# revdotcom/reverb

Measured on AMD Instinct MI355X. Metric: RTFx (audio-sec/wall-sec) Reverb-ASR attention_rescoring, higher is better.
Workload: dtype bf16

## Files before the change

### reverb_amd/_lib.py

```python
from __future__ import annotations

import ctypes as C
import os

_HERE = os.path.dirname(os.path.abspath(__file__))
LIB_PATH = os.path.join(_HERE, "librvb.so")

RVB_F32, RVB_BF16, RVB_FP8 = 0, 1, 2
ACT_NONE, ACT_SILU, ACT_RELU = 0, 1, 2
NORM_LN, NORM_AFFINE = 0, 1


class RvbError(RuntimeError):
    pass


class AudioInfo(C.Structure):
    _fields_ = [("container", C.c_int32), ("sample_format", C.c_int32), ("channels", C.c_int32), ("sample_rate", C.c_int32),
                ("bits_per_sample", C.c_int32), ("md5_checked", C.c_int32), ("frames", C.c_int64), ("decode_threads", C.c_int32),
                ("reserved", C.c_int32)]


class _SizedCfg(C.Structure):

# ... 115 lines not shown
                [("p", _f32p), ("p_rows", C.c_int32), ("p_stride", C.c_int32), ("p_col", C.c_int32), ("p_off", C.c_int32),
                 ("bias_u", _f32p), ("bias_v", _f32p)] +
                [(n, _i32p) for n in ("q_start", "q_len", "kv_start", "kv_len", "q_pos0", "kv_index", "work")] +
                [(n, C.c_int32) for n in ("n_index", "n_work", "max_q", "q_block", "causal", "chunk", "left", "plain_order", "fold",
                                          "k_prefolded", "fold_kv_cap", "lab")] +
                [("ran", C.c_int32 * 8)])


class NormTestArgs(C.Structure):
    _fields_ = ([(n, C.c_int32) for n in ("dtype", "x_bf16", "mode", "silu", "out_f32", "out_fp8", "out2_fp8", "M", "d", "pad0")] +
                [(n, C.c_float) for n in ("eps", "eps2", "out_scale", "out2_scale")] +
                [(n, _f32p) for n in ("x", "gamma", "beta", "add", "gamma2", "beta2", "out", "out2")] +
                [("sat", C.c_uint32), ("sat2", C.c_uint32)])


class GemmTestArgs(C.Structure):
    _fields_ = ([(n, C.c_int32) for n in ("dtype", "M", "N", "K", "lda", "ldw", "ldc", "ldres", "act", "out_f32", "out_fp8", "in_fp8",
                                          "inplace", "a_row0", "c_rows", "conv", "cT1", "cF1", "cC", "cB")] +
                [(n, C.c_float) for n in ("alpha", "a_scale", "out_scale")] +
                [("path", C.c_int32), ("a_elems", C.c_int64)] +
                [(n, _f32p) for n in ("A", "W", "bias", "res", "C", "a_deq", "w_deq")])


_u32p = C.POINTER(C.c_uint32)

TEST_SIGNATURES = {
    "rvb_test_gemm_ex": (C.c_int, [C.POINTER(GemmTestArgs)]),
    "rvb_test_rownorm_ex": (C.c_int, [C.POINTER(NormTestArgs)]),
    "rvb_test_conv1_ex": (C.c_int, [C.c_int, _f32p, _f32p, _f32p, _f32p, _f32p, _f32p, C.c_int, C.c_int, C.c_int, C.c_int, C.c_float,
                                    _f32p, _u32p]),
    "rvb_test_embed": (C.c_int, [_f32p, C.c_int, _f32p, C.c_int, _i32p, _i32p, _f32p, C.c_int, C.c_int, C.c_float]),
    "rvb_test_amax_abs": (C.c_int, [C.c_int, _f32p, C.c_int64, _f32p]),
    "rvb_test_convert_f32": (C.c_int, [C.c_int, _f32p, _f32p, C.c_int64]),
    "rvb_test_gather_cache": (C.c_int, [C.c_void_p, C.c_void_p, _i32p, C.c_int, C.c_int, C.c_int, C.c_int]),
    "rvb_test_gather_pairs": (C.c_int, [_f32p, C.c_int, C.c_int64, _i32p, _i32p, C.c_int, _f32p]),
    "rvb_test_gemm": (C.c_int, [C.c_int, _f32p, _f32p, _f32p, _f32p, _f32p, C.c_int, C.c_int, C.c_int, C.c_float,
                                C.c_int, C.c_int, C.c_int, C.c_int, C.c_int, C.c_int, C.c_int]),
    "rvb_test_rownorm": (C.c_int, [C.c_int, _f32p, _f32p, _f32p, C.c_float, C.c_int, C.c_int, _f32p, _f32p, C.c_int,
                                   C.c_int, C.c_int]),
    "rvb_test_conv_block32": (C.c_int, [_f32p, _f32p, _f32p, _f32p, _f32p, _f32p, C.c_int, C.c_int, C.c_int]),
    "rvb_test_conv_s2sc": (C.c_int, [_f32p, _f32p, _f32p, _f32p, _f32p, _f32p, _f32p, C.c_int, C.c_int, C.c_int]),
    "rvb_test_conv1": (C.c_int, [C.c_int, _f32p, _f32p, _f32p, _f32p, _f32p, _f32p, C.c_int, C.c_int, C.c_int, C.c_int]),
    "rvb_test_conv_igemm_fp8": (C.c_int, [_f32p, _f32p, _f32p, _f32p, _f32p, _f32p, C.c_int, C.c_int, C.c_int, C.c_int, C.c_int, C.c_int, C.c_int,
                                           C.c_float, C.c_float, _f32p, _f32p, _f32p]),
    "rvb_test_joint_new": (C.c_void_p, [C.c_int, C.c_int, C.c_int, C.c_int, C.c_double, C.c_double, C.c_double]),
    "rvb_test_joint_free": (None, [C.c_void_p]),
    "rvb_test_joint_begin": (C.c_int, [C.c_void_p, C.c_int, _f32p, _i32p, C.c_int, C.c_float, C.c_float, _i32p, _i32p, _i32p, _i32p, _i32p,
                                       C.c_int]),
    "rvb_test_joint_finish": (C.c_int, [C.c_void_p, _f32p]),
    "rvb_test_joint_prefix": (C.c_int, [C.c_void_p, C.c_int, _i32p, _i32p]),
    "rvb_test_joint_result": (C.c_int, [C.c_void_p, _i32p, _i32p, _i32p, _f64p, _i32p, _f64p]),
    "rvb_test_glu_dwconv": (C.c_int, [C.c_int, _f32p, _f32p, _f32p, _f32p, _i32p, _f32p, C.c_int, C.c_int, C.c_int,
                                      C.c_int, C.c_int, _f32p, C.c_int]),
    "rvb_test_attention": (C.c_int, [C.c_int, _f32p, _f32p, _f32p, _f32p, _f32p, _f32p, _f32p, C.c_int, C.c_int,
                                     C.c_int, C.c_int, C.c_int, _i32p, _i32p, _i32p, _i32p, C.c_int, C.c_int]),
    "rvb_test_attention_trie": (C.c_int, [C.c_int, _f32p, _f32p, _f32p, _f32p, C.c_int, C.c_int, C.c_int, _i32p, _i32p, _i32p,
                                          _i32p, _i32p, _i32p, C.c_int, C.c_int, C.c_int]),
    "rvb_test_attention_ex": (C.c_int, [C.POINTER(AttnTestArgs)]),
    "rvb_test_attention_pos_bias": (C.c_int, [_f32p, C.c_int, C.c_int, C.c_int, C.c_int, _f32p, _f32p, C.c_int, C.c_int, C.c_float, _f32p]),
    "rvb_test_logsoftmax_topk": (C.c_int, [_f32p, C.c_int, C.c_int, C.c_int, C.c_float, C.c_int, _f32p, _i32p, _f32p]),
    "rvb_test_lse_gather": (C.c_int, [_f32p, C.c_int, C.c_int, _i32p, _f32p]),
    "rvb_test_logsoftmax_topk_ex": (C.c_int, [_f32p, C.c_int, C.c_int, C.c_int, C.c_int, C.c_float, C.c_int, _f32p, _i32p, _f32p]),
    "rvb_test_lse_gather_ex": (C.c_int, [_f32p, C.c_int, C.c_int, C.c_int, _i32p, C.c_float, C.c_int, _f32p]),
    "rvb_test_lse_gather_multi_ex": (C.c_int, [_f32p, C.c_int, C.c_int, C.c_int, _i32p, _i32p, _f32p]),
    "rvb_test_ctc_viterbi": (C.c_int, [_f32p, C.c_int, C.c_int, _i32p, C.c_int, C.c_int, C.c_int, _i32p, _f32p]),
    "rvb_test_ctc_viterbi_wild": (C.c_int, [_f32p, C.c_int, C.c_int, _f32p, C.c_float, _i32p, C.c_int, C.c_int, C.c_int, _i32p, _f32p]),
    "rvb_test_ctc_viterbi_graph": (C.c_int, [_f32p, _i32p, C.c_int, C.c_int, _f32p, C.c_float, _i32p, _i32p, _i32p, _i32p, _u8p, C.c_int,
                                             C.c_int, _i32p, _i32p, _f32p]),
    "rvb_test_ctc_score": (C.c_int, [_f32p, C.c_int, C.c_int, _i32p, C.c_int, C.c_int, C.c_int, _f64p, _f32p, _f32p, _f32p, _i32p]),
    "rvb_test_ctc_score_graph": (C.c_int, [_f32p, _i32p, C.c_int, C.c_int, _i32p, _i32p, _i32p, _i32p, _u8p, C.c_int, C.c_int, _f64p, _f32p,
                                           _f32p, _f32p, _f32p, _i32p]),
    "rvb_test_ctc_score_batch": (C.c_int, [_f32p, _i32p, C.c_int, _i32p, _i32p, C.c_int, C.c_int, C.c_int, _f64p, _f32p, _f32p, _f32p,
                                           _i32p]),
    "rvb_test_ctc_find": (C.c_int, [_f32p, _i32p, C.c_int, C.c_int, _f32p, _i32p, _i32p, C.c_int, _f32p, C.c_int, C.c_int, C.c_int, C.c_int,
                                    _i64p, _i32p, _i32p, _f32p, _i32p, _i32p, _i32p, _f32p]),
    "rvb_test_slab_windows": (C.c_int, [C.c_char_p, _i32p, _i32p, C.c_int, _i32p, C.c_int, C.c_int, _i32p, _i32p, _i32p, _i32p, _i32p]),
    "rvb_test_gemm_glu": (C.c_int, [_f32p, _f32p, _f32p, _f32p, C.c_int, C.c_int, C.c_int]),
    "rvb_test_gemm_rowadd": (C.c_int, [_f32p, _f32p, _f32p, _f32p, _f32p, C.c_int, C.c_int, C.c_int, C.c_int, C.c_int, C.c_int]),
    "rvb_test_mp3_decode": (C.c_int64, [C.c_char_p, C.c_int64, C.c_int, _f32p, C.c_int64, _i64p, _i64p, C.c_int]),
    "rvb_test_mp3_hybrid": (C.c_int, [_f32p, _f32p, C.c_int, C.c_int, _f32p]),
    "rvb_test_mp3_polyphase": (C.c_int, [_f32p, _f32p, _i32p, _f32p]),
    "rvb_test_mp3_window": (C.c_int, [_f32p]),
    "rvb_test_mp3_huffman": (C.c_int, [C.c_int, C.POINTER(C.c_uint16), C.POINTER(C.c_uint8), _i32p]),
    "rvb_test_gemm_fp8": (C.c_int, [_f32p, _f32p, _f32p, _f32p, _f32p, C.c_int, C.c_int, C.c_int, C.c_float, C.c_float, C.c_int, C.c_int,
                                    C.c_float, _f32p, _f32p]),
    "rvb_test_rownorm_fp8": (C.c_int, [_f32p, _f32p, _f32p, C.c_float, C.c_int, C.c_int, C.c_int, C.c_float, _f32p, _f32p, _f32p,
                                       C.c_float, C.c_float, _f32p, _f32p]),
    "rvb_test_lse_gather_multi": (C.c_int, [_f32p, C.c_int, C.c_int, _i32p, _i32p, C.c_int, _f32p]),
    "rvb_test_row_xent": (C.c_int, [_f32p, C.c_int, C.c_int, C.c_int, _i32p, _i32p, _f32p, _f32p, _f64p, _i32p]),
    "rvb_test_host_pool": (C.c_int, [C.c_int, C.c_int, C.c_int]),
    "rvb_test_build_trie": (C.c_int, [_i32p, _i32p, _i32p, C.c_int, C.c_int, C.c_int, C.c_int, C.c_int, _i32p, _i32p, _i32p, _i32p, _i32p, _i32p,
                                      _i32p, _i32p, _i32p, _i32p, _i32p]),
    "rvb_test_fbank": (C.c_int, [_i16p, C.c_int64, _f32p]),
    "rvb_test_fbank_ex": (C.c_int, [_i16p, _f32p, C.c_int64, _f32p]),
    "rvb_test_fbank_batch": (C.c_int, [C.POINTER(C.c_void_p), _i32p, _i64p, _i64p, C.c_int, C.c_int, _f32p]),
    "rvb_test_set_gemm_variant": (C.c_int, [C.c_int]),
    "rvb_test_set_gemm2_opts": (C.c_int, [C.c_int, C.c_int]),
    "rvb_test_gemm_timeline": (C.c_int, [C.c_int] * 6 + [C.POINTER(C.c_longlong), C.c_int, _i32p]),
    "rvb_test_gemm_bench": (C.c_int, [C.c_int, C.c_int, C.c_int, C.c_int, C.c_int, C.c_int, C.c_int, C.c_int, C.c_int,
                                      _f64p, _f64p]),
    "rvb_test_prefix_beam": (C.c_int, [_f32p, _i32p, C.c_int, C.c_int, C.c_int, _i32p, _i32p, _i32p, _i32p, _i32p,
                                       _f64p]),
    "rvb_test_prefix_beam_context": (C.c_int, [_f32p, _i32p, C.c_int, C.c_int, C.c_int, C.c_int, _i32p, _i32p, C.c_int, C.c_double,
                                               _i32p, _i32p, _i32p, _i32p, _i32p, _f64p, _f64p]),
    "rvb_test_context_walk": (C.c_int, [_i32p, _i32p, C.c_int, C.c_double, C.c_int, C.c_int, _i32p, C.c_int, _i32p, _f64p, _i32p,
                                        _f64p]),
# ... 127 lines not shown
```

### reverb_amd/csrc/elementwise.hip

```cpp
#include <algorithm>

#include "common.h"
#include "kernels.h"

namespace rvb {

static constexpr int CONV1_ROWS = 4;

template <typename T>
__global__ __launch_bounds__(256) void conv1_kernel(const float* __restrict__ feats, const float* __restrict__ mean,
                                                    const float* __restrict__ istd, const float* __restrict__ w,
                                                    const float* __restrict__ bias, T* __restrict__ out, int T0,
                                                    int F0, int T1, int F1, int d, float inv_scale, unsigned* __restrict__ amax,
                                                    unsigned* __restrict__ sat) {
  extern __shared__ float s_in[];
  const int t1_0 = blockIdx.x * CONV1_ROWS, b = blockIdx.y;
  const int nrow = min(CONV1_ROWS, T1 - t1_0);
  for (int i = threadIdx.x; i < (2 * nrow + 1) * F0; i += 256) {
    const int kh = i / F0, f = i - kh * F0;
    s_in[i] = (feats[((size_t)b * T0 + 2 * t1_0 + kh) * F0 + f] - mean[f]) * istd[f];
  }
  __syncthreads();
  const int ncg = d >> 3;
  const int per = ncg < 256 ? ncg : 256;
  const int nslots = 256 / per;
  const int cgl = threadIdx.x % per, fslot = threadIdx.x / per;
  if (fslot >= nslots) return;
  float vmax = 0.f;
  unsigned nclip = 0;
  for (int cg = cgl; cg < ncg; cg += per) {
    float wr[8][9], br[8];
#pragma unroll
    for (int k = 0; k < 9; ++k) {
      const float4 lo = *(const float4*)(w + (size_t)k * d + cg * 8), hi = *(const float4*)(w + (size_t)k * d + cg * 8 + 4);
      wr[0][k] = lo.x; wr[1][k] = lo.y; wr[2][k] = lo.z; wr[3][k] = lo.w;
      wr[4][k] = hi.x; wr[5][k] = hi.y; wr[6][k] = hi.z; wr[7][k] = hi.w;
    }
#pragma unroll
    for (int c = 0; c < 8; ++c) br[c] = bias[cg * 8 + c];
    for (int row = 0; row < nrow; ++row) {
      T* orow = out + ((size_t)b * T1 + t1_0 + row) * F1 * d;
      const float* in = s_in + 2 * row * F0;
      for (int f1 = fslot; f1 < F1; f1 += nslots) {
        float xin[9];
#pragma unroll
        for (int kh = 0; kh < 3; ++kh)
#pragma unroll
          for (int kw = 0; kw < 3; ++kw) xin[kh * 3 + kw] = in[kh * F0 + 2 * f1 + kw];
        float o[8];
        if constexpr (sizeof(T) == 4) {
#pragma unroll
          for (int c = 0; c < 8; ++c) {
            float acc = br[c];
// ... 416 lines not shown
    for (int e = 0; e < VE; ++e) sv[e] = Gate<T>::put(g[e]);
    uint4* dst = (uint4*)&s_g[r][grp * VE];
#pragma unroll
    for (int q = 0; q < (int)(VE * sizeof(S)) / 16; ++q) dst[q] = ((const uint4*)sv)[q];
  }
  }
  __syncthreads();
  if (!cok) return;
  constexpr int OPT = DW_TT / (DW_THREADS / 64);
  f32x2_t acc[OPT];
  const f32x2_t bv = {a.dw_b[ch], a.dw_b[ch + 1]};
#pragma unroll
  for (int i = 0; i < OPT; ++i) acc[i] = bv;
  const int rbase = slot * OPT;
#pragma unroll
  for (int r = 0; r < OPT + DW_KMAX - 1; ++r) {
    float gx, gy;
    Gate<T>::get(*(const typename Gate<T>::pair_t*)&s_g[rbase + r][2 * c], gx, gy);
    const f32x2_t g = {gx, gy};
#pragma unroll
    for (int i = 0; i < OPT; ++i) {
      const int k = r - i;
      if (k >= 0 && k < DW_KMAX) acc[i] = __builtin_elementwise_fma(wk[k], g, acc[i]);
    }
  }
#pragma unroll
  for (int i = 0; i < OPT; ++i) {
    const int t = t0 + rbase + i;
    if (t < a.T) {
      if (a.out_bf16) *(uint32_t*)((bf16_t*)a.out + ((size_t)b * a.T + t) * a.d + ch) = pack2_bf16(acc[i].x, acc[i].y);
      else *(float2*)(a.out + ((size_t)b * a.T + t) * a.d + ch) = make_float2(acc[i].x, acc[i].y);
    }
  }
}

int glu_dwconv(hipStream_t s, int dtype, const GluDwArgs& a) {
  if (a.B <= 0 || a.T <= 0) return OK;
  if (a.K > DW_KMAX || a.K < 1 || (!a.causal && (a.K % 2) == 0) || (a.d % 2)) {
    set_error("glu_dwconv: kernel must be <= 31 (and odd unless causal), d even"); return E_ARG;
  }
  if (a.gated && (a.hist_rows > 0 || (a.d % (dtype == DT_BF16 ? 8 : 4)) != 0)) {
    set_error("glu_dwconv: a gated input comes in whole 16-byte vectors and without a streaming history"); return E_ARG;
  }
  if (a.hist_rows > 0 && (!a.causal || a.B != 1 || a.hist_rows > a.K - 1 || !a.hist)) {
    set_error("glu_dwconv: a left-context history belongs to one causal stream"); return E_ARG;
  }
  dim3 grid(cdiv(a.T, DW_TT), cdiv(a.d, DW_CT), a.B);
  if (dtype == DT_BF16) hipLaunchKernelGGL(glu_dw_kernel<bf16_t>, grid, dim3(DW_THREADS), 0, s, a);
  else hipLaunchKernelGGL(glu_dw_kernel<float>, grid, dim3(DW_THREADS), 0, s, a);
  RVB_HIP_CHECK(hipGetLastError());
  return OK;
}

__global__ __launch_bounds__(256) void embed_kernel(const float* __restrict__ E, const float* __restrict__ pe,
                                                    const int* __restrict__ tok, const int* __restrict__ pos,
                                                    float* __restrict__ out, int rows, int d, float scale) {
  const int row = blockIdx.x;
  const float* e = E + (size_t)tok[row] * d;
  const float* p = pe + (size_t)pos[row] * d;
  for (int c = threadIdx.x; c < d; c += 256) out[(size_t)row * d + c] = e[c] * scale + p[c];
}

int embed_tokens(hipStream_t s, const float* E, const float* pe, const int* tok, const int* pos, float* out,
                 int rows, int d, float scale) {
  if (rows <= 0) return OK;
  hipLaunchKernelGGL(embed_kernel, dim3(rows), dim3(256), 0, s, E, pe, tok, pos, out, rows, d, scale);
  RVB_HIP_CHECK(hipGetLastError());
  return OK;
}

template <typename T>
__global__ __launch_bounds__(256) void amax_kernel(const T* __restrict__ x, size_t n, float* __restrict__ slot) {
  float m = 0.f;
  for (size_t i = (size_t)blockIdx.x * 256 + threadIdx.x; i < n; i += (size_t)gridDim.x * 256) m = fmaxf(m, fabsf(Cvt<T>::to_f32(x[i])));
  m = wave_max(m);
  if ((threadIdx.x & 63) == 0 && m > 0.f) atomicMax((unsigned int*)slot, __float_as_uint(m));
}
int amax_abs(hipStream_t s, int dtype, const void* x, size_t n, float* slot) {
  if (n == 0) return OK;
  const int blocks = (int)std::min<size_t>((n + 255) / 256, 2048);
  if (dtype == DT_BF16) hipLaunchKernelGGL(amax_kernel<bf16_t>, dim3(blocks), dim3(256), 0, s, (const bf16_t*)x, n, slot);
  else hipLaunchKernelGGL(amax_kernel<float>, dim3(blocks), dim3(256), 0, s, (const float*)x, n, slot);
  RVB_HIP_CHECK(hipGetLastError());
  return OK;
}

template <typename T>
__global__ __launch_bounds__(256) void convert_kernel(const float* __restrict__ src, T* __restrict__ dst, size_t n) {
  for (size_t i = (size_t)blockIdx.x * 256 + threadIdx.x; i < n; i += (size_t)gridDim.x * 256)
    dst[i] = Cvt<T>::from_f32(src[i]);
}

int convert_f32(hipStream_t s, int dtype, const float* src, void* dst, size_t n) {
  if (n == 0) return OK;
  const int blocks = (int)((n + 255) / 256 < 4096 ? (n + 255) / 256 : 4096);
  if (dtype == DT_BF16) hipLaunchKernelGGL(convert_kernel<bf16_t>, dim3(blocks), dim3(256), 0, s, src, (bf16_t*)dst, n);
  else hipLaunchKernelGGL(convert_kernel<float>, dim3(blocks), dim3(256), 0, s, src, (float*)dst, n);
  RVB_HIP_CHECK(hipGetLastError());
  return OK;
}

__global__ __launch_bounds__(256) void gather_cache_kernel(const char* __restrict__ src, char* __restrict__ dst,
                                                           const int* __restrict__ parent, int L, int rows, int row_bytes) {
  const int r = blockIdx.y;
  const size_t so = (size_t)parent[r] * L * row_bytes, dof = (size_t)r * L * row_bytes;
  const int nvec = rows * (row_bytes / 16);
// ... 15 lines not shown
```

### reverb_amd/csrc/engine_encode.hip

```cpp
#include "engine_impl.h"

#include <algorithm>
#include <cmath>
#include <cstdlib>
#include <cstring>

namespace rvb {

static constexpr int GLU_FUSE_DEFAULT = 1;

static int encoder_layer(rvb_engine* e, EncLayer& L, int lidx, int M, int B, int T, const LNorm& next, void* next_out,
                         float next8 = 0.f, int li = -1) {
  const int d = e->cfg.d_model, ff = e->cfg.ffn_dim, heads = e->cfg.heads, dk = d / heads;
  float* x = e->x.as<float>();
  const bool f8 = e->fp8 && e->f8_state == 2 && li < 0;
  const bool cal = e->fp8 && e->f8_state == 1 && li < 0;
  const unsigned grp = f8 ? e->f8_groups[lidx] : 0u;
  const bool f8_ffm = grp & 1u, f8_qkv = grp & 2u, f8_pw1 = grp & 4u, f8_pw2 = grp & 8u, f8_ff = (grp & 16u) && !L.is_lsl;
  const F8Scales sc8 = f8 ? e->f8[lidx] : F8Scales();
  const char* prefold_env = lab_env("RVB_ATTN_PREFOLD");
  const int prefold_on = prefold_env ? atoi(prefold_env) : 1;
  const bool prefold = prefold_on && e->dtype == DT_BF16 && li < 0 && !f8_qkv && L.pos_bias.p != nullptr && dk > 32 && dk <= 64 &&
                       T <= e->pe_rows && T <= 16384 && (d % 8) == 0;
  auto note = [&](int slot, const void* t, size_t n) -> int {
// ... 37 lines not shown
      static const int fold = lab_env("RVB_ATTN_FOLD") ? atoi(lab_env("RVB_ATTN_FOLD")) : 0;
      const int cap = (T + 63) / 64 * 64;
      if (fold && li < 0 && L.pos_bias.p && cap <= 16384) { a.pos_bias = L.pos_bias.as<float>(); a.pos_bias_stride = e->pe_rows; a.fold_kv_cap = cap; }
      if (prefold && cap <= 16384) { a.pos_bias = L.pos_bias.as<float>(); a.pos_bias_stride = e->pe_rows; a.k_prefolded = 1; a.fold_kv_cap = cap; }
    }
    a.q_stride = a.k_stride = a.v_stride = 3 * d; a.p_stride = d; a.o_stride = d;
    a.bias_u = L.bias_u.as<float>(); a.bias_v = L.bias_v.as<float>();
    a.out = e->ao.p;
    a.q_start = e->d_seq_start.as<int>(); a.q_len = e->d_seq_len.as<int>();
    a.kv_start = e->d_seq_start.as<int>(); a.kv_len = e->cur_lens;
    a.nseq = B; a.heads = heads; a.dk = dk; a.max_q = T; a.causal = 0; a.sqrt_dk = std::sqrt((float)dk);
    a.chunk = e->dec_chunk; a.left = e->dec_left;
    { static const int qb = lab_env("RVB_ATTN_QBLOCK") ? atoi(lab_env("RVB_ATTN_QBLOCK")) : 0; a.q_block = qb; }
    double keys = T;
    if (li >= 0) {
      auto& st = e->stream_st;
      char* kvb = (char*)st.kv[li].p;
      RVB_HIP_CHECK(hipMemcpy2DAsync(kvb + (size_t)st.cache_len * 2 * d * es, (size_t)2 * d * es, (const char*)e->h.p + (size_t)d * es,
                                     (size_t)3 * d * es, (size_t)2 * d * es, M, hipMemcpyDeviceToDevice, e->stream));
      a.k = kvb; a.v = kvb + (size_t)d * es; a.k_stride = a.v_stride = 2 * d;
      a.p = (const char*)L.pos_keys.p + (size_t)(st.offset - st.cache_len) * d * es;
      if (a.pos_bias) a.pos_bias += (st.offset - st.cache_len);
      a.kv_start = e->d_stream_i32.as<int>(); a.kv_len = e->d_stream_i32.as<int>() + 1;
      a.chunk = 0; a.left = -1;
      keys = st.cache_len + M;
    }
    Scope sc(e, "attention", 6.0 * B * (double)T * keys * d);
    RVB_TRY(attention(e->stream, e->dtype, with_lab(a)));
  }
  RVB_TRY(run_gemm(e, e->ao.p, d, L.att_out, x, d, M, true, 1.f, ACT_NONE, x, d));
  bool glu_fused = false;
  if (f8_pw1) {
    RVB_TRY(run_norm(e, x, L.n_conv, e->xn.p, false, M, d, NORM_LN, 0, nullptr, nullptr, nullptr, sc8.in_pw1, 0.f, false, satp(3)));
    RVB_TRY(run_gemm8(e, e->xn.p, d, L.pw1, e->h.p, 2 * d, M, sc8.in_pw1, 0));
  } else {
    RVB_TRY(run_norm(e, x, L.n_conv, e->xn.p, false, M, d));
    RVB_TRY(note(3, e->xn.p, (size_t)M * d));
    {
      const char* ge = lab_env("RVB_GLU_FUSE");
      const int glu_on = ge ? atoi(ge) : GLU_FUSE_DEFAULT;
      GemmArgs t;
      memset(&t, 0, sizeof(t));
      t.A = e->xn.p; t.W = L.pw1_glu.w.p; t.bias = L.pw1_glu.b.as<float>(); t.C = e->h.p; t.M = M; t.N = 2 * d; t.K = d; t.lda = d; t.ldw = d;
      t.ldc = d; t.alpha = 1.f; t.act = ACT_GLU;
      glu_fused = glu_on && li < 0 && L.pw1_glu.w.p != nullptr && !cal && gemm_glu_supported(e->dtype, t);
      if (glu_fused) {
        Scope sc(e, "gemm", 2.0 * M * (double)t.N * t.K, gemm_alg_bytes(e, t));
        RVB_TRY(gemm(e->stream, e->dtype, t));
      } else {
        RVB_TRY(run_gemm(e, e->xn.p, d, L.pw1, e->h.p, 2 * d, M, false));
      }
    }
  }
  {
    GluDwArgs g;
    g.gated = glu_fused ? 1 : 0;
    g.G = e->h.p; g.pw1_bias = L.pw1.b.as<float>(); g.dw_w = L.dw_w.as<float>(); g.dw_b = L.dw_b.as<float>();
    g.lens = e->cur_lens; g.out = e->dconv.as<float>(); g.B = B; g.T = T; g.d = d; g.K = e->cfg.cnn_kernel;
    g.causal = e->cfg.cnn_causal ? 1 : 0;
    g.out_bf16 = e->dtype == DT_BF16 ? 1 : 0;
    const int lorder = g.K - 1;
    const bool cached = li >= 0 && g.causal && lorder > 0;
    if (cached) { g.hist = e->stream_st.cnn[li].p; g.hist_rows = e->stream_st.cnn_rows; }
    {
      Scope sc(e, "glu_dwconv");
      RVB_TRY(glu_dwconv(e->stream, e->dtype, g));
    }
    if (cached) {
      auto& st = e->stream_st;
      const size_t es = dt_size(e->dtype), rb = (size_t)2 * d * es;
      if (M >= lorder) {
        RVB_HIP_CHECK(hipMemcpyAsync(st.cnn[li].p, (const char*)e->h.p + (size_t)(M - lorder) * rb, (size_t)lorder * rb,
                                     hipMemcpyDeviceToDevice, e->stream));
      } else {
        RVB_HIP_CHECK(hipMemcpyAsync(st.cnn2[li].p, (const char*)st.cnn[li].p + (size_t)M * rb, (size_t)(lorder - M) * rb,
                                     hipMemcpyDeviceToDevice, e->stream));
        RVB_HIP_CHECK(hipMemcpyAsync((char*)st.cnn2[li].p + (size_t)(lorder - M) * rb, e->h.p, (size_t)M * rb,
                                     hipMemcpyDeviceToDevice, e->stream));
        std::swap(st.cnn[li], st.cnn2[li]);
      }
    }
  }
  const int cmode = e->cfg.cnn_norm == 0 ? NORM_LN : NORM_AFFINE;
  const bool dw16 = e->dtype == DT_BF16;
  if (f8_pw2) {
    RVB_TRY(run_norm(e, e->dconv.as<float>(), L.n_cnn, e->xn.p, false, M, d, cmode, 1, nullptr, nullptr, nullptr, sc8.in_pw2, 0.f, dw16, satp(4)));
    RVB_TRY(run_gemm8(e, e->xn.p, d, L.pw2, x, d, M, sc8.in_pw2, 1, 1.f, 1.f, ACT_NONE, x, d));
  } else {
    RVB_TRY(run_norm(e, e->dconv.as<float>(), L.n_cnn, e->xn.p, false, M, d, cmode, 1, nullptr, nullptr, nullptr, 0.f, 0.f, dw16));
    RVB_TRY(note(4, e->xn.p, (size_t)M * d));
    RVB_TRY(run_gemm(e, e->xn.p, d, L.pw2, x, d, M, true, 1.f, ACT_NONE, x, d));
  }
  if (f8_ff) {
    RVB_TRY(run_norm(e, x, L.n_ff, e->xn.p, false, M, d, NORM_LN, 0, nullptr, nullptr, nullptr, sc8.in_ff1, 0.f, false, satp(5)));
    RVB_TRY(run_gemm8(e, e->xn.p, d, L.ff1, e->h.p, ff, M, sc8.in_ff1, 2, sc8.h_ff, 1.f, ACT_SILU, nullptr, 0, satp(6)));
    RVB_TRY(run_gemm8(e, e->h.p, ff, L.ff2, x, d, M, sc8.h_ff, 1, 1.f, 0.5f, ACT_NONE, x, d));
  } else {
    RVB_TRY(run_norm(e, x, L.n_ff, e->xn.p, false, M, d));
    const void* ffin = e->xn.p;
    if (L.is_lsl) {
      RVB_TRY(run_gemm(e, e->xn.p, d, L.lsl, e->y.p, d, M, false));
      ffin = e->y.p;
    } else {
      RVB_TRY(note(5, e->xn.p, (size_t)M * d));
    }
    RVB_TRY(run_gemm(e, ffin, d, L.ff1, e->h.p, ff, M, false, 1.f, ACT_SILU));
    if (!L.is_lsl) RVB_TRY(note(6, e->h.p, (size_t)M * ff));
    RVB_TRY(run_gemm(e, e->h.p, ff, L.ff2, x, d, M, true, 0.5f, ACT_NONE, x, d));
  }
  RVB_TRY(run_norm(e, x, L.n_final, x, true, M, d, NORM_LN, 0, L.is_lsl ? e->y.p : nullptr, &next, next_out, 0.f, f8 ? next8 : 0.f, false,
                   nullptr, (f8 && next8 > 0.f && e->d_f8sat.p) ? e->d_f8sat.as<unsigned>() + (size_t)(lidx + 1) * 8 : nullptr));
  return OK;
}

int encode_impl(rvb_engine* e, const float* feats, int64_t first_chunk, const int32_t* lens, int B, int T0,
                       int beam, float blank_penalty) {
  const rvb_model_cfg& c = e->cfg;
  if (!e->finalized) { set_error("rvb_encode before rvb_finalize"); return E_STATE; }
  if (B <= 0 || B > c.max_chunks || T0 < 7 || T0 > c.chunk_frames) {
    set_error("rvb_encode: need 1 <= B <= max_chunks and 7 <= T0 <= chunk_frames"); return E_ARG;
  }
  if (beam < 1 || beam > 64 || beam > c.vocab) { set_error("rvb_encode: beam must be in [1,64]"); return E_ARG; }
  RVB_HIP_CHECK(hipSetDevice(e->device));
  RVB_TRY(wait_slices(e, -1));
  e->stream_st.active = false;
  const int d = c.d_model, F0 = c.input_dim, V = c.vocab;
  const int T1 = (T0 - 3) / 2 + 1, F1 = (F0 - 3) / 2 + 1, T2 = (T1 - 3) / 2 + 1, F2 = (F1 - 3) / 2 + 1;
  const int M = B * T2;
  const size_t es = dt_size(e->dtype);
  e->B = B; e->T0 = T0; e->T1 = T1; e->F1 = F1; e->T2 = T2; e->F2 = F2; e->beam = beam;
  e->dec_l.kv_ready = e->dec_r.kv_ready = false;
  e->last_blank_penalty = blank_penalty;
  e->in_lens.assign(lens, lens + B);
  e->enc_lens.resize(B);
  std::vector<int32_t> starts(B), qlens(B, T2);
  for (int b = 0; b < B; ++b) {
    if (lens[b] < 0 || lens[b] > T0) { set_error("rvb_encode: lens out of range"); return E_ARG; }
    e->enc_lens[b] = lens[b] > 6 ? (lens[b] - 7) / 4 + 1 : 0;
// ... 278 lines not shown
```

### reverb_amd/csrc/kernels.h

```cpp
#pragma once
#include <vector>
#include "common.h"

namespace rvb {

enum { DT_F32 = 0, DT_BF16 = 1 };
enum { ACT_NONE = 0, ACT_SILU = 1, ACT_RELU = 2, ACT_LRELU = 3  };
enum { ACT_GLU = 4 };

inline size_t dt_size(int dt) { return dt == DT_BF16 ? 2 : 4; }

struct GemmArgs {
  const void* A;
  const void* W;
  const float* bias;
  const float* res;
  void* C;
  int M, N, K;
  int lda, ldw, ldc, ldres;
  float alpha;
  int act;
  int out_f32;
  int conv;
  int cT1, cF1, cT2, cF2, cC;
// ... 36 lines not shown
                int64_t total_frames, float* feats, int64_t n_rows, const FbankTables& t);
void resample_taps(int sample_rate, int target, std::vector<float>* ker, int* orig, int* new_, int* width, int* K);
int round_to_i16(hipStream_t s, const float* x, int64_t n, int16_t* out);
int resample(hipStream_t s, const int16_t* pcm, int64_t n_in, const float* ker, int orig, int new_, int width, int K, float* out,
             int64_t n_out);
int resample_f32(hipStream_t s, const float* wave, int64_t n_in, const float* ker, int orig, int new_, int width, int K, float* out,
             int64_t n_out);

int subsample_conv1(hipStream_t s, int dtype, const float* feats, const float* mean, const float* istd,
                    const float* w , const float* b , void* out, int B, int T0, int F0,
                    int d, float out_fp8_scale = 0.f , unsigned* amax = nullptr ,
                    unsigned* sat = nullptr );

enum { NORM_LN = 0, NORM_AFFINE = 1 };
struct NormArgs {
  const float* x;
  int x_bf16 = 0;
  const float* gamma;
  const float* beta;
  float eps;
  int mode;
  int silu;
  const void* add;
  void* out;
  int out_f32;
  int M, d;
  const float* gamma2 = nullptr;
  const float* beta2 = nullptr;
  float eps2 = 0.f;
  void* out2 = nullptr;
  int out_fp8 = 0, out2_fp8 = 0;
  float out_inv_scale = 1.f, out2_inv_scale = 1.f;
  unsigned* sat = nullptr;
  unsigned* sat2 = nullptr;
};
int rownorm(hipStream_t s, int dtype, const NormArgs& a);

struct GluDwArgs {
  const void* G;
  const float* pw1_bias;
  const float* dw_w;
  const float* dw_b;
  const int* lens;
  float* out;
  int B, T, d, K;
  int out_bf16 = 0;
  int gated = 0;
  int causal = 0;
  const void* hist = nullptr;
  int hist_rows = 0;
};
int glu_dwconv(hipStream_t s, int dtype, const GluDwArgs& a);

int embed_tokens(hipStream_t s, const float* E, const float* pe, const int* tok, const int* pos, float* out,
                 int rows, int d, float scale);

int logsoftmax_topk(hipStream_t s, const float* logits, int M, int V, int ld, int k, float blank_penalty,
                    int blank_id, float* topk_val, int* topk_idx, float* logp_out);

int lse_gather(hipStream_t s, const float* logits, int R, int V, int ld, const int* target, float* out, float blank_penalty = 0.f,
               int blank_id = -1);
int lse_gather_multi(hipStream_t s, const float* logits, int R, int V, int ld, const int* ptr, const int* target, float* out);
int row_xent(hipStream_t s, const float* logits, int R, int V, int ld, const int* ptr, const int* target, float* logp, float* lse,
             double* sum_x, int* top1);

int gather_pairs(hipStream_t s, const float* table, size_t ld, const int* row, const int* col, int n, float* out);

int gather_cache(hipStream_t s, const void* src, void* dst, const int* parent, int R, int L, int rows, int row_bytes);

int amax_abs(hipStream_t s, int dtype, const void* x, size_t n, float* slot);

int convert_f32(hipStream_t s, int dtype, const float* src, void* dst, size_t n);

enum { CTC_ALIGN_MAX_TOKENS = 16383,
       CTC_ALIGN_MAX_STATES = 2 * CTC_ALIGN_MAX_TOKENS + 1,
       CTC_ALIGN_MAX_FRAMES = 1 << 20 };
inline int ctc_spt_for(int S) { return S <= 4096 ? 4 : S <= 16384 ? 16 : 32; }
inline int ctc_threads(int n, int per_thread) { const int t = ((n + per_thread - 1) / per_thread + 63) / 64 * 64; return t < 1024 ? t : 1024; }
struct VitSeq {
  int L, S, T;
  int tok_off;
  int frame_off;
  int f0, f1;
  int pad_;
  long long alpha_off;
  long long bp_off;
  long long bp_stride;
};
int ctc_viterbi_forward(hipStream_t s, const VitSeq* seqs, int n_seq, int max_S, const float* lp, int ld, int r0, const int* rows,
                        const int* tokens, int blank, float* alpha, uint8_t* bp, const float* wmax = nullptr, float bias = 0.f);
int ctc_viterbi_backtrace(hipStream_t s, const VitSeq* seqs, int n_seq, const float* alpha, const uint8_t* bp, int* states, float* score);

enum { CTC_GRAPH_MAX_NODES = 8192,
       CTC_GRAPH_MAX_IN_DEGREE = 64,
       CTC_GRAPH_MAX_ARCS = 32768 };
struct GraphSeq {
  int N, T;
  int index;
  int node_off;
  int arc_off;
  int frame_off;
  int fin_off, n_final;
  int f0, f1;
  long long alpha_off;
  long long bp_off;
  long long bp_stride;
// ... 192 lines not shown
```

Measured before the change: 27900.

## Fuse depthwise conv with conformer conv-module norm and SiLU into one kernel

Adds a bf16 kernel that does the gated depthwise convolution over time tiles and then, in the same workgroup, the LayerNorm or affine norm and SiLU on each row. It writes bf16 directly as the input to the pw2 GEMM. This removes the fp32 dconv intermediate round-trip and a separate norm launch. It is enabled by default through an env flag, applies only for 512<d<=1024, bf16, non-fp8 and non-calibration paths, and adds a test binding. The cost is a complex hand-scheduled kernel that keeps the conv result in bf16 before the norm, which changes numerics slightly.

```diff
diff --git a/reverb_amd/_lib.py b/reverb_amd/_lib.py
--- a/reverb_amd/_lib.py
+++ b/reverb_amd/_lib.py
@@ -191,6 +191,8 @@
     "rvb_test_joint_result": (C.c_int, [C.c_void_p, _i32p, _i32p, _i32p, _f64p, _i32p, _f64p]),
     "rvb_test_glu_dwconv": (C.c_int, [C.c_int, _f32p, _f32p, _f32p, _f32p, _i32p, _f32p, C.c_int, C.c_int, C.c_int,
                                       C.c_int, C.c_int, _f32p, C.c_int]),
+    "rvb_test_dw_norm": (C.c_int, [C.c_int, _f32p, _f32p, _f32p, _f32p, _i32p, _f32p, _f32p, C.c_float, C.c_int, _f32p, C.c_int, C.c_int,
+                                   C.c_int, C.c_int, C.c_int]),
     "rvb_test_attention": (C.c_int, [C.c_int, _f32p, _f32p, _f32p, _f32p, _f32p, _f32p, _f32p, C.c_int, C.c_int,
                                      C.c_int, C.c_int, C.c_int, _i32p, _i32p, _i32p, _i32p, C.c_int, C.c_int]),
     "rvb_test_attention_trie": (C.c_int, [C.c_int, _f32p, _f32p, _f32p, _f32p, C.c_int, C.c_int, C.c_int, _i32p, _i32p, _i32p,
diff --git a/reverb_amd/csrc/elementwise.hip b/reverb_amd/csrc/elementwise.hip
--- a/reverb_amd/csrc/elementwise.hip
+++ b/reverb_amd/csrc/elementwise.hip
@@ -1,4 +1,5 @@
 #include <algorithm>
+#include <type_traits>
 
 #include "common.h"
 #include "kernels.h"
@@ -521,6 +522,171 @@
   return OK;
 }
 
+static constexpr int DN_TT = 16, DN_ROWS = DN_TT + DW_KMAX - 1, DN_FIRST = 4, DN_AHEAD = 8, DN_AHEAD_EDGE = 8, DN_STEP = 4, DN_MAX_THREADS = 512;
+
+template <bool LN>
+__global__ __launch_bounds__(DN_MAX_THREADS, 4) void dw_norm_kernel(DwNormArgs a, int tpc, int tpw, int ntiles) {
+  extern __shared__ __attribute__((aligned(16))) uint32_t s_dn[];
+  const int lane = __lane_id(), wave = __builtin_amdgcn_readfirstlane(threadIdx.x >> 6), nw = blockDim.x >> 6;
+  const int d = a.d, T = a.T;
+  const int ch = 2 * (int)threadIdx.x;
+  const bool cok = ch < d;
+  const int chl = min(ch, d - 2);
+  const int K = a.K, pad = a.causal ? K - 1 : (K - 1) / 2;
+  typedef float f32x2_t __attribute__((ext_vector_type(2)));
+  const unsigned off2 = (unsigned)chl * 2u, off4 = (unsigned)chl * 4u;
+  typedef const __attribute__((address_space(1))) char* gchar_p;
+  f32x2_t wk[DW_KMAX];
+#pragma unroll
+  for (int k = 0; k < DW_KMAX; ++k) {
+    gchar_p row = (gchar_p)((const char*)a.dw_w + (size_t)min(k, K - 1) * d * sizeof(float));
+    asm volatile("" : "+s"(row));
+    wk[k] = *(const __attribute__((address_space(1))) f32x2_t*)(row + off4);
+  }
+#pragma unroll
+  for (int k = 0; k < DW_KMAX; ++k) {
+    asm volatile("" : "+v"(wk[k]));
+    wk[k] = k < K ? wk[k] : (f32x2_t){0.f, 0.f};
+  }
+  const f32x2_t bv = {a.dw_b[chl], a.dw_b[chl + 1]};
+  const uint32_t bg = (uint32_t)f32_to_bf16(a.pw1_bias[chl] / (1.0f + expf(-a.pw1_bias[d + chl]))) |
+                      ((uint32_t)f32_to_bf16(a.pw1_bias[chl + 1] / (1.0f + expf(-a.pw1_bias[d + chl + 1]))) << 16);
+  float* s_gb = (float*)(s_dn + 2 * DN_TT * (d >> 1));
+  for (int c = 4 * (int)threadIdx.x; c < 2 * d; c += 4 * (int)blockDim.x)
+    *(float4*)(s_gb + c) = c < d ? *(const float4*)(a.gamma + c) : *(const float4*)(a.beta + (c - d));
+  const int first = blockIdx.x * tpw, last = min(first + tpw, ntiles);
+  for (int tile = first; tile < last; ++tile) {
+    const int b = tile / tpc, t0 = (tile - b * tpc) * DN_TT;
+    const int len = max(min(a.lens[b], T), 0);
+    unsigned o2 = off2;
+    asm volatile("" : "+v"(o2));
+    const char* Gb = (const char*)((const bf16_t*)a.G + (size_t)b * T * d);
+    auto ld = [&](int r) __attribute__((always_inline)) {
+      gchar_p row = (gchar_p)(Gb + (size_t)min(max(t0 - pad + r, 0), T - 1) * d * sizeof(bf16_t));
+      asm volatile("" : "+s"(row));
+      return *(const __attribute__((address_space(1))) uint32_t*)(row + o2);
+    };
+    uint32_t raw[DN_ROWS];
+#pragma unroll
+    for (int r = 0; r < DN_FIRST; ++r) raw[r] = ld(r);
+    f32x2_t acc[DN_TT];
+#pragma unroll
+    for (int i = 0; i < DN_TT; ++i) acc[i] = bv;
+    auto conv = [&](auto edge) __attribute__((always_inline)) {
+      constexpr int AHEAD = decltype(edge)::value ? DN_AHEAD_EDGE : DN_AHEAD;
+#pragma unroll
+      for (int r = 0; r < DN_ROWS; ++r) {
+        if (r % DN_STEP == 0) {
+          __builtin_amdgcn_sched_barrier(0);
+#pragma unroll
+          for (int q = (r == 0 ? DN_FIRST : max(DN_FIRST, r + AHEAD - DN_STEP)); q < r + AHEAD && q < DN_ROWS; ++q) raw[q] = ld(q);
+          __builtin_amdgcn_sched_barrier(0);
+        }
+        uint32_t u = raw[r];
+        if constexpr (decltype(edge)::value) {
+          const int t = t0 - pad + r;
+          const int below = t < 0, frame = (unsigned)t < (unsigned)len;
+          const int filled = (below & (a.causal != 0)) | (~below & ~frame & (t < T));
+          u = (u & (uint32_t)-frame) | (bg & (uint32_t)-(filled & 1));
+        }
+        const f32x2_t g = {__uint_as_float(u << 16), __uint_as_float(u & 0xffff0000u)};
+#pragma unroll
+        for (int i = 0; i < DN_TT; ++i) {
+          const int k = r - i;
+          if (k >= 0 && k < DW_KMAX) acc[i] = __builtin_elementwise_fma(wk[k], g, acc[i]);
+        }
+      }
+    };
+    if (t0 - pad >= 0 && t0 - pad + DN_ROWS <= len) conv(std::false_type());
+    else conv(std::true_type());
+    __builtin_amdgcn_sched_barrier(0);
+#define COL(i) ((((lane) + 64 * ((i) >> 1)) << 3) + (((i) & 1) << 2))
+    constexpr int NV = 4;
+    uint32_t* s_t = s_dn + ((tile - first) & 1) * (DN_TT * (d >> 1));
+    if (cok) {
+#pragma unroll
+      for (int i = 0; i < DN_TT; ++i) s_t[i * (d >> 1) + (o2 >> 2)] = pack2_bf16(acc[i].x, acc[i].y);
+    }
+    __syncthreads();
+    for (int row = wave; row < DN_TT; row += nw) {
+      const int t = t0 + row;
+      if (t >= T) break;
+      const bf16_t* x = (const bf16_t*)s_t + row * d;
+      float4 v[NV];
+#pragma unroll
+      for (int i = 0; i < NV; i += 2) {
+        const int c = COL(i);
+        const uint4 u = *(const uint4*)(x + min(c, d - 8));
+        const bool ok = c < d;
+        v[i] = make_float4(ok ? bf16_to_f32((bf16_t)(u.x & 0xffffu)) : 0.f, ok ? bf16_to_f32((bf16_t)(u.x >> 16)) : 0.f,
+                           ok ? bf16_to_f32((bf16_t)(u.y & 0xffffu)) : 0.f, ok ? bf16_to_f32((bf16_t)(u.y >> 16)) : 0.f);
+        v[i + 1] = make_float4(ok ? bf16_to_f32((bf16_t)(u.z & 0xffffu)) : 0.f, ok ? bf16_to_f32((bf16_t)(u.z >> 16)) : 0.f,
+                               ok ? bf16_to_f32((bf16_t)(u.w & 0xffffu)) : 0.f, ok ? bf16_to_f32((bf16_t)(u.w >> 16)) : 0.f);
+      }
+      float mean = 0.f, rstd = 1.f;
+      if constexpr (LN) {
+        float sum = 0.f;
+#pragma unroll
+        for (int i = 0; i < NV; ++i) sum += v[i].x + v[i].y + v[i].z + v[i].w;
+        mean = wave_sum_dpp(sum) / (float)d;
+        float sq = 0.f;
+#pragma unroll
+        for (int i = 0; i < NV; ++i) {
+          if (COL(i) < d) {
+            sq += sq4<NV>(v[i].x - mean, v[i].y - mean, v[i].z - mean, v[i].w - mean);
+          }
+        }
+        rstd = rsqrtf(wave_sum_dpp(sq) / (float)d + a.eps);
+      }
+      bf16_t* out = (bf16_t*)a.out + ((size_t)b * T + t) * d;
+#pragma unroll
+      for (int i = 0; i < NV; ++i) {
+        const int c = COL(i);
+        if (c >= d) continue;
+        const float4 g = *(const float4*)(s_gb + c), be = *(const float4*)(s_gb + d + c);
+        float o[4] = {(v[i].x - mean) * rstd * g.x + be.x, (v[i].y - mean) * rstd * g.y + be.y,
+                      (v[i].z - mean) * rstd * g.z + be.z, (v[i].w - mean) * rstd * g.w + be.w};
+#pragma unroll
+        for (int e = 0; e < 4; ++e) o[e] = o[e] * __builtin_amdgcn_rcpf(1.0f + __builtin_amdgcn_exp2f(-1.44269504f * o[e]));
+        v[i] = make_float4(o[0], o[1], o[2], o[3]);
+      }
+#pragma unroll
+      for (int i = 0; i < NV; i += 2) {
+        const int c = COL(i);
+        if (c >= d) continue;
+        *(uint4*)(out + c) = make_uint4(pack2_bf16(v[i].x, v[i].y), pack2_bf16(v[i].z, v[i].w),
+                                        pack2_bf16(v[i + 1].x, v[i + 1].y), pack2_bf16(v[i + 1].z, v[i + 1].w));
+      }
+    }
+#undef COL
+  }
+}
+
+bool dw_norm_supported(int dtype, const DwNormArgs& a) {
+  return dtype == DT_BF16 && a.gated && a.hist_rows == 0 && a.K >= 1 && a.K <= DW_KMAX && (a.causal || (a.K % 2) == 1) &&
+         a.d > 512 && a.d <= 1024 && (a.d % 8) == 0 && (a.mode == NORM_LN || a.mode == NORM_AFFINE);
+}
+
+int dw_norm(hipStream_t s, int dtype, const DwNormArgs& a) {
+  if (!dw_norm_supported(dtype, a)) {
+    set_error("dw_norm: bf16 engine, gated input, no streaming history, kernel <= 31 (odd unless causal), 512 < d <= 1024, d % 8 == 0");
+    return E_ARG;
+  }
+  if (a.B <= 0 || a.T <= 0) return OK;
+  static const int slots = [] { int dev = 0, cus = 0; if (hipGetDevice(&dev) != hipSuccess || hipDeviceGetAttribute(&cus, hipDeviceAttributeMultiprocessorCount, dev) != hipSuccess || cus <= 0) cus = 256; return 2 * cus; }();
+  const int tpc = cdiv(a.T, DN_TT), ntiles = tpc * a.B;
+  const int tpw = a.tiles_per_wg > 0 ? a.tiles_per_wg : std::max(1, cdiv(ntiles, slots));
+  const dim3 grid(cdiv(ntiles, tpw)), block(cdiv(a.d, 128) * 64);
+  const size_t sh = (size_t)2 * DN_TT * a.d * sizeof(bf16_t) + (size_t)2 * a.d * sizeof(float);
+  if (sh > 64 * 1024)
+    RVB_HIP_CHECK(hipFuncSetAttribute(a.mode == NORM_LN ? (const void*)dw_norm_kernel<true> : (const void*)dw_norm_kernel<false>,
+                                      hipFuncAttributeMaxDynamicSharedMemorySize, (int)sh));
+  if (a.mode == NORM_LN) hipLaunchKernelGGL(dw_norm_kernel<true>, grid, block, sh, s, a, tpc, tpw, ntiles);
+  else hipLaunchKernelGGL(dw_norm_kernel<false>, grid, block, sh, s, a, tpc, tpw, ntiles);
+  RVB_HIP_CHECK(hipGetLastError());
+  return OK;
+}
+
 __global__ __launch_bounds__(256) void embed_kernel(const float* __restrict__ E, const float* __restrict__ pe,
                                                     const int* __restrict__ tok, const int* __restrict__ pos,
                                                     float* __restrict__ out, int rows, int d, float scale) {
diff --git a/reverb_amd/csrc/engine_encode.hip b/reverb_amd/csrc/engine_encode.hip
--- a/reverb_amd/csrc/engine_encode.hip
+++ b/reverb_amd/csrc/engine_encode.hip
@@ -113,7 +113,21 @@
       }
     }
   }
-  {
+  const int cmode = e->cfg.cnn_norm == 0 ? NORM_LN : NORM_AFFINE;
+  bool dw_norm_fused = false;
+  if (glu_fused && !f8_pw2 && !cal) {
+    const char* fe = lab_env("RVB_DW_NORM_FUSE");
+    DwNormArgs n;
+    n.G = e->h.p; n.pw1_bias = L.pw1.b.as<float>(); n.dw_w = L.dw_w.as<float>(); n.dw_b = L.dw_b.as<float>();
+    n.lens = e->cur_lens; n.B = B; n.T = T; n.d = d; n.K = e->cfg.cnn_kernel; n.causal = e->cfg.cnn_causal ? 1 : 0;
+    n.gamma = L.n_cnn.g.as<float>(); n.beta = L.n_cnn.b.as<float>(); n.eps = L.n_cnn.eps; n.mode = cmode; n.out = e->xn.p;
+    dw_norm_fused = (fe ? atoi(fe) : 1) && dw_norm_supported(e->dtype, n);
+    if (dw_norm_fused) {
+      Scope sc(e, "glu_dwconv");
+      RVB_TRY(dw_norm(e->stream, e->dtype, n));
+    }
+  }
+  if (!dw_norm_fused) {
     GluDwArgs g;
     g.gated = glu_fused ? 1 : 0;
     g.G = e->h.p; g.pw1_bias = L.pw1.b.as<float>(); g.dw_w = L.dw_w.as<float>(); g.dw_b = L.dw_b.as<float>();
@@ -142,9 +156,10 @@
       }
     }
   }
-  const int cmode = e->cfg.cnn_norm == 0 ? NORM_LN : NORM_AFFINE;
   const bool dw16 = e->dtype == DT_BF16;
-  if (f8_pw2) {
+  if (dw_norm_fused) {
+    RVB_TRY(run_gemm(e, e->xn.p, d, L.pw2, x, d, M, true, 1.f, ACT_NONE, x, d));
+  } else if (f8_pw2) {
     RVB_TRY(run_norm(e, e->dconv.as<float>(), L.n_cnn, e->xn.p, false, M, d, cmode, 1, nullptr, nullptr, nullptr, sc8.in_pw2, 0.f, dw16, satp(4)));
     RVB_TRY(run_gemm8(e, e->xn.p, d, L.pw2, x, d, M, sc8.in_pw2, 1, 1.f, 1.f, ACT_NONE, x, d));
   } else {
diff --git a/reverb_amd/csrc/kernels.h b/reverb_amd/csrc/kernels.h
--- a/reverb_amd/csrc/kernels.h
+++ b/reverb_amd/csrc/kernels.h
@@ -112,6 +112,27 @@
 };
 int glu_dwconv(hipStream_t s, int dtype, const GluDwArgs& a);
 
+struct DwNormArgs {
+  const void* G;
+  const float* pw1_bias;
+  const float* dw_w;
+  const float* dw_b;
+  const int* lens;
+  int B, T, d, K;
+  int gated = 1;
+  int causal = 0;
+  const void* hist = nullptr;
+  int hist_rows = 0;
+  const float* gamma;
+  const float* beta;
+  float eps;
+  int mode;
+  void* out;
+  int tiles_per_wg = 0;
+};
+bool dw_norm_supported(int dtype, const DwNormArgs& a);
+int dw_norm(hipStream_t s, int dtype, const DwNormArgs& a);
+
 int embed_tokens(hipStream_t s, const float* E, const float* pe, const int* tok, const int* pos, float* out,
                  int rows, int d, float scale);
 
```

Result: no change. 28080 (median of 2 runs) (+0.7%).
